# ActiveVisionLab/gaussctrl

Hardware: AMD Instinct MI355X
Metric: edited views/sec @512x512 (ControlNet denoise + splat render+bwd) (higher is better)
Workload: dtype bf16

## Files before the change

### gaussctrl_amd/csrc/dn_gemm_kernels.h

```cpp
#pragma once
#include "dn_common.h"
#include <type_traits>

namespace dng {
struct GemmArgs {
    int64_t M, N, K;
    const void *A; int64_t lda;
    int B, Hi, Wi, Cin, Ho, Wo, stride, ups, pad;
    const void *W;
    const float *bias;
    const float *rowvec; int64_t ld_rowvec; int64_t rows_per_batch;
    const void *residual; int64_t ldr;
    float out_scale;
    int act, geglu;
    void *out; int64_t ldc; int out_f32;
    void *out_t; int64_t ldt; int64_t t_batch_stride; int64_t t_col0;
    int splits; int tiles_per_split;
    int persist;
    float *ws;
    const void *zeros;
    const float *row_stats; int row_stat_slots; const float *colsum; float ln_eps, ln_inv_k;
    float *out_row_stats;
    float *out_group_stats;
    int gn_groups, gn_cpg;
// ... 887 lines not shown
            }
            block(f1, f0, st1, 0, more, tnone, std::false_type{}, w3_tag);
            st = st1;
        }
    };
    if (w3) run(std::true_type{}); else run(std::false_type{});

    if constexpr (FUSE) {
        wave_epilogue<T, NTW, MT, 512>(g, acc, m_base, m_base + wm * (16 * MT), n_base + wn * (16 * NTW), lane, smem,
                                       (g.row_stats && g.splits == 1) ? srow : nullptr, slice);
        return;
    }
    const int64_t n_lane = n_base + wn * (16 * NTW) + fc * 4;
    if (g.splits > 1) {
#pragma unroll
        for (int mt = 0; mt < MT; ++mt) {
            const int64_t m = m_base + wm * (16 * MT) + mt * 16 + fr;
            if (m >= g.M) continue;
#pragma unroll
            for (int nt = 0; nt < NTW; ++nt) {
                const int64_t n = n_lane + nt * 16;
                if (n < g.N)
                    *reinterpret_cast<float4 *>(g.ws + ((int64_t)slice * g.M + m) * g.N + n) =
                        make_float4(acc[nt][mt][0], acc[nt][mt][1], acc[nt][mt][2], acc[nt][mt][3]);
            }
        }
        return;
    }
    if constexpr (LNV == 3) {
        const float *biasp = g.bias + wset * g.N, *csp = g.colsum + wset * g.N;
        float4 bia[NTW], csm[NTW];
#pragma unroll
        for (int nt = 0; nt < NTW; ++nt) {
            const int64_t n = n_lane + nt * 16, nc = n < g.N ? n : g.N - 4;
            bia[nt] = *reinterpret_cast<const float4 *>(biasp + nc);
            csm[nt] = *reinterpret_cast<const float4 *>(csp + nc);
        }
#pragma unroll
        for (int mt = 0; mt < MT; ++mt) {
            const int64_t m = m_base + wm * (16 * MT) + mt * 16 + fr;
            const float2 st = *reinterpret_cast<const float2 *>(srow + 2 * (wm * (16 * MT) + mt * 16 + fr));
            const float mean = st.x * g.ln_inv_k, rstd = rsqrtf(fmaxf(st.y * g.ln_inv_k - mean * mean, 0.f) + g.ln_eps);
            float v[NTW][4];
            float mx = -3.0e38f;
#pragma unroll
            for (int nt = 0; nt < NTW; ++nt) {
                v[nt][0] = rstd * (acc[nt][mt][0] - mean * csm[nt].x) + bia[nt].x; v[nt][1] = rstd * (acc[nt][mt][1] - mean * csm[nt].y) + bia[nt].y;
                v[nt][2] = rstd * (acc[nt][mt][2] - mean * csm[nt].z) + bia[nt].z; v[nt][3] = rstd * (acc[nt][mt][3] - mean * csm[nt].w) + bia[nt].w;
#pragma unroll
                for (int r = 0; r < 4; ++r) {
                    const bool key = nt * 16 + fc * 4 + r < g.sm_keys;
                    v[nt][r] = key ? v[nt][r] : -3.0e38f;
                    mx = fmaxf(mx, v[nt][r]);
                }
            }
            mx = fmaxf(mx, __shfl_xor(mx, 16, 64)); mx = fmaxf(mx, __shfl_xor(mx, 32, 64));
            float sum = 0.f;
#pragma unroll
            for (int nt = 0; nt < NTW; ++nt)
#pragma unroll
                for (int r = 0; r < 4; ++r) { v[nt][r] = exp2f(v[nt][r] - mx); sum += v[nt][r]; }
            sum += __shfl_xor(sum, 16, 64); sum += __shfl_xor(sum, 32, 64);
            const float inv = 1.f / sum;
#pragma unroll
            for (int nt = 0; nt < NTW; ++nt) {
                const int64_t n = n_lane + nt * 16;
                if (m < g.M && n < g.N)
                    *reinterpret_cast<uint2 *>((unsigned char *)g.out + (m * g.ldc + n) * 2) =
                        make_uint2(pack2<T>(v[nt][0] * inv, v[nt][1] * inv), pack2<T>(v[nt][2] * inv, v[nt][3] * inv));
            }
        }
        return;
    }
    if constexpr (LEAN) {
        const unsigned char *zp = (const unsigned char *)g.zeros;
        const bool has_b = g.bias != nullptr, has_rv = g.rowvec != nullptr, has_res = g.residual != nullptr;
        const float *biasp = has_b ? g.bias + (LNV != 0 ? wset * g.N : 0) : reinterpret_cast<const float *>(zp);
        const float *rvp = has_rv ? g.rowvec : reinterpret_cast<const float *>(zp);
        const unsigned char *resp = has_res ? (const unsigned char *)g.residual : zp;
        const int64_t bA = m_base / g.rows_per_batch, b_last = (g.M - 1) / g.rows_per_batch;
        const int64_t bB = bA + 1 < b_last ? bA + 1 : b_last;
        const int64_t m_rv = (bA + 1) * g.rows_per_batch;
        float4 bia[NTW], rvA[NTW], rvB[NTW];
        uint2 rs[MT][NTW];
#pragma unroll
        for (int nt = 0; nt < NTW; ++nt) {
            const int64_t n = n_lane + nt * 16, nc = n < g.N ? n : g.N - 4;
            bia[nt] = *reinterpret_cast<const float4 *>(biasp + (has_b ? nc : 0));
            rvA[nt] = *reinterpret_cast<const float4 *>(rvp + (has_rv ? bA * g.ld_rowvec + nc : 0));
            rvB[nt] = *reinterpret_cast<const float4 *>(rvp + (has_rv ? bB * g.ld_rowvec + nc : 0));
        }
#pragma unroll
        for (int mt = 0; mt < MT; ++mt) {
            const int64_t m = m_base + wm * (16 * MT) + mt * 16 + fr, mc = m < g.M ? m : g.M - 1;
#pragma unroll
            for (int nt = 0; nt < NTW; ++nt) {
                const int64_t n = n_lane + nt * 16, nc = n < g.N ? n : g.N - 4;
                rs[mt][nt] = *reinterpret_cast<const uint2 *>(resp + (has_res ? (mc * g.ldr + nc) * 2 : 0));
            }
        }
        float4 csm[LNV == 2 ? NTW : 1];
        if constexpr (LNV == 2) {
#pragma unroll
            for (int nt = 0; nt < NTW; ++nt) {
                const int64_t n = n_lane + nt * 16, nc = n < g.N ? n : g.N - 4;
                csm[nt] = *reinterpret_cast<const float4 *>(g.colsum + wset * g.N + nc);
            }
        }
        uint2 pks[CS ? MT : 1][CS ? NTW : 1];
#pragma unroll
        for (int mt = 0; mt < MT; ++mt) {
            const int64_t m = m_base + wm * (16 * MT) + mt * 16 + fr;
            const bool second = m >= m_rv;
            float mean = 0.f, rstd = 1.f;
            if constexpr (LNV == 2) {
                const float2 st = *reinterpret_cast<const float2 *>(srow + 2 * (wm * (16 * MT) + mt * 16 + fr));
                mean = st.x * g.ln_inv_k;
                rstd = rsqrtf(fmaxf(st.y * g.ln_inv_k - mean * mean, 0.f) + g.ln_eps);
            }
            float rsum = 0.f, rsq = 0.f;
#pragma unroll
            for (int nt = 0; nt < NTW; ++nt) {
                const int64_t n = n_lane + nt * 16;
                const float4 rv = second ? rvB[nt] : rvA[nt];
                float a0 = acc[nt][mt][0], a1 = acc[nt][mt][1], a2 = acc[nt][mt][2], a3 = acc[nt][mt][3];
                if constexpr (LNV == 2) {
                    a0 = rstd * (a0 - mean * csm[nt].x); a1 = rstd * (a1 - mean * csm[nt].y);
                    a2 = rstd * (a2 - mean * csm[nt].z); a3 = rstd * (a3 - mean * csm[nt].w);
                }
                float v[4] = {a0 + bia[nt].x + rv.x, a1 + bia[nt].y + rv.y, a2 + bia[nt].z + rv.z, a3 + bia[nt].w + rv.w};
#pragma unroll
                for (int r = 0; r < 4; ++r) v[r] *= g.out_scale;
                v[0] += T::to_f((unsigned short)(rs[mt][nt].x & 0xffff)); v[1] += T::to_f((unsigned short)(rs[mt][nt].x >> 16));
                v[2] += T::to_f((unsigned short)(rs[mt][nt].y & 0xffff)); v[3] += T::to_f((unsigned short)(rs[mt][nt].y >> 16));
                const uint2 pk = make_uint2(pack2<T>(v[0], v[1]), pack2<T>(v[2], v[3]));
                const bool ok = m < g.M && n < g.N;
                if (ok) *reinterpret_cast<uint2 *>((unsigned char *)g.out + (m * g.ldc + n) * 2) = pk;
                if constexpr (CS) pks[mt][nt] = ok ? pk : make_uint2(0u, 0u);
                if constexpr (LNV == 1) {
                    const float w_ = n < g.N ? 1.f : 0.f;
                    const float t0 = w_ * T::to_f((unsigned short)(pk.x & 0xffff)), t1 = w_ * T::to_f((unsigned short)(pk.x >> 16));
                    const float t2 = w_ * T::to_f((unsigned short)(pk.y & 0xffff)), t3 = w_ * T::to_f((unsigned short)(pk.y >> 16));
                    rsum += (t0 + t1) + (t2 + t3); rsq += (t0 * t0 + t1 * t1) + (t2 * t2 + t3 * t3);
                }
            }
            if constexpr (LNV == 1) {
                rsum += __shfl_xor(rsum, 16, 64); rsq += __shfl_xor(rsq, 16, 64);
                rsum += __shfl_xor(rsum, 32, 64); rsq += __shfl_xor(rsq, 32, 64);
                const int64_t slot = (n_base + wn * (16 * NTW)) / (16 * NTW);
                if (fc == 0 && m < g.M && n_base + wn * (16 * NTW) < g.N)
                    *reinterpret_cast<float2 *>(g.out_row_stats + (slot * g.M + m) * 2) = make_float2(rsum, rsq);
            }
        }
        if constexpr (CS) {
            const int64_t m_split = (m_base / g.rows_per_batch + 1) * g.rows_per_batch;
            const int64_t m_end = m_base + BM < g.M ? m_base + BM : g.M;
            const int npass = m_split < m_end ? 2 : 1;
    #pragma unroll 1
            for (int pass = 0; pass < npass; ++pass) {
                float cs[NTW][4], cq[NTW][4];
    #pragma unroll
                for (int nt = 0; nt < NTW; ++nt)
    #pragma unroll
                    for (int r = 0; r < 4; ++r) { cs[nt][r] = 0.f; cq[nt][r] = 0.f; }
    #pragma unroll
                for (int mt = 0; mt < MT; ++mt) {
                    const int64_t m_tile = m_base + wm * (16 * MT) + mt * 16;
                    const float wgt = ((m_tile >= m_split ? 1 : 0) == pass) ? 1.f : 0.f;
    #pragma unroll
                    for (int nt = 0; nt < NTW; ++nt) {
                        const uint2 pk = pks[mt][nt];
                        const float t0 = wgt != 0.f ? T::to_f((unsigned short)(pk.x & 0xffff)) : 0.f, t1 = wgt != 0.f ? T::to_f((unsigned short)(pk.x >> 16)) : 0.f;
                        const float t2 = wgt != 0.f ? T::to_f((unsigned short)(pk.y & 0xffff)) : 0.f, t3 = wgt != 0.f ? T::to_f((unsigned short)(pk.y >> 16)) : 0.f;
                        cs[nt][0] += t0; cq[nt][0] += t0 * t0; cs[nt][1] += t1; cq[nt][1] += t1 * t1;
                        cs[nt][2] += t2; cq[nt][2] += t2 * t2; cs[nt][3] += t3; cq[nt][3] += t3 * t3;
                    }
                }
                float *tb = ctab + (pass * BN + wn * (16 * NTW) + fc * 4) * 2;
    #pragma unroll
                for (int nt = 0; nt < NTW; ++nt)
    #pragma unroll
                    for (int r = 0; r < 4; ++r) {
                        const float sa = row16_sum(cs[nt][r]), sb = row16_sum(cq[nt][r]);
                        if (fr == 0) {
                            __hip_atomic_fetch_add(tb + (nt * 16 + r) * 2, sa, __ATOMIC_RELAXED, __HIP_MEMORY_SCOPE_WORKGROUP);
                            __hip_atomic_fetch_add(tb + (nt * 16 + r) * 2 + 1, sb, __ATOMIC_RELAXED, __HIP_MEMORY_SCOPE_WORKGROUP);
                        }
                    }
            }
            asm volatile("s_waitcnt lgkmcnt(0)" ::: "memory");
            __builtin_amdgcn_s_barrier();
            const int64_t b0 = m_base / g.rows_per_batch;
            const int cpg = g.gn_cpg, G = (int)(g.N / cpg);
            const int n_hi = (int)(n_base + BN < g.N ? n_base + BN : g.N);
            const int g_first = (int)n_base / cpg, ng = (n_hi - 1) / cpg - g_first + 1;
            for (int i = tid; i < 2 * ng; i += 512) {
                const int slot = i >= ng ? 1 : 0, gg = g_first + i - slot * ng;
                if (slot == 1 && !(m_split < m_end)) continue;
                const int c_lo = gg * cpg > (int)n_base ? gg * cpg : (int)n_base, c_hi = (gg + 1) * cpg < n_hi ? (gg + 1) * cpg : n_hi;
                float s1 = 0.f, s2 = 0.f;
                for (int c = c_lo; c < c_hi; ++c) { const float2 t = *reinterpret_cast<const float2 *>(ctab + (slot * BN + c - (int)n_base) * 2); s1 += t.x; s2 += t.y; }
                const int64_t b = b0 + slot;
                const int64_t slab = mblk - (b * g.rows_per_batch) / BM;
                const int half = gg * cpg < (int)n_base ? 1 : 0;
                *reinterpret_cast<float2 *>(g.chan_parts + ((((b * g.cp_nslab + slab) * G + gg) * 2 + half) * 2)) = make_float2(s1, s2);
            }
        }
    } else {
    float4 bia[NTW], csm[LNV == 2 ? NTW : 1];
#pragma unroll
    for (int nt = 0; nt < NTW; ++nt) {
        const int64_t n = n_lane + nt * 16;
        bia[nt] = (g.bias && n < g.N) ? *reinterpret_cast<const float4 *>(g.bias + n) : make_float4(0.f, 0.f, 0.f, 0.f);
        if constexpr (LNV == 2) csm[nt] = n < g.N ? *reinterpret_cast<const float4 *>(g.colsum + n) : make_float4(0.f, 0.f, 0.f, 0.f);
    }
#pragma unroll
    for (int mt = 0; mt < MT; ++mt) {
        const int64_t m = m_base + wm * (16 * MT) + mt * 16 + fr;
        if (m >= g.M) continue;
        if constexpr (LNV == 2) {
            const float2 st = *reinterpret_cast<const float2 *>(srow + 2 * (wm * (16 * MT) + mt * 16 + fr));
            const float mean = st.x * g.ln_inv_k, rstd = rsqrtf(fmaxf(st.y * g.ln_inv_k - mean * mean, 0.f) + g.ln_eps);
#pragma unroll
            for (int nt = 0; nt < NTW; ++nt) {
                acc[nt][mt][0] = rstd * (acc[nt][mt][0] - mean * csm[nt].x); acc[nt][mt][1] = rstd * (acc[nt][mt][1] - mean * csm[nt].y);
                acc[nt][mt][2] = rstd * (acc[nt][mt][2] - mean * csm[nt].z); acc[nt][mt][3] = rstd * (acc[nt][mt][3] - mean * csm[nt].w);
            }
        }
        float4 rv[NTW];
        uint2 rs[NTW];
        const int64_t bidx = g.rowvec ? m / g.rows_per_batch : 0;
#pragma unroll
        for (int nt = 0; nt < NTW; ++nt) {
            const int64_t n = n_lane + nt * 16;
            const bool okn = n < g.N && !(g.geglu && (nt & 1));
            const int64_t on = g.geglu ? (n_base + wn * (16 * NTW) + nt * 16) / 2 + fc * 4 : n;
            rv[nt] = (g.rowvec && n < g.N) ? *reinterpret_cast<const float4 *>(g.rowvec + bidx * g.ld_rowvec + n) : make_float4(0.f, 0.f, 0.f, 0.f);
            rs[nt] = (g.residual && okn) ? *reinterpret_cast<const uint2 *>((const unsigned char *)g.residual + (m * g.ldr + on) * 2) : make_uint2(0u, 0u);
        }
#pragma unroll
        for (int nt = 0; nt < NTW; ++nt) {
            const int64_t n = n_lane + nt * 16;
            if (n >= g.N) continue;
            if (g.geglu && (nt & 1)) continue;
            float v[4] = {acc[nt][mt][0] + bia[nt].x + rv[nt].x, acc[nt][mt][1] + bia[nt].y + rv[nt].y,
                          acc[nt][mt][2] + bia[nt].z + rv[nt].z, acc[nt][mt][3] + bia[nt].w + rv[nt].w};
            int64_t on = n;
            if (g.geglu) {
                constexpr int NP = NTW - 1;
                const int np = nt + 1 < NTW ? nt + 1 : NP;
                v[0] *= gelu_erf(acc[np][mt][0] + bia[np].x); v[1] *= gelu_erf(acc[np][mt][1] + bia[np].y);
                v[2] *= gelu_erf(acc[np][mt][2] + bia[np].z); v[3] *= gelu_erf(acc[np][mt][3] + bia[np].w);
                on = (n_base + wn * (16 * NTW) + nt * 16) / 2 + fc * 4;
            }
            if (g.act == 1) {
#pragma unroll
                for (int r = 0; r < 4; ++r) v[r] = silu(v[r]);
            } else if (g.act == 2) {
#pragma unroll
                for (int r = 0; r < 4; ++r) v[r] = fminf(fmaxf(v[r] * 0.5f + 0.5f, 0.f), 1.f);
            }
#pragma unroll
            for (int r = 0; r < 4; ++r) v[r] *= g.out_scale;
            if (g.residual) {
                v[0] += T::to_f((unsigned short)(rs[nt].x & 0xffff)); v[1] += T::to_f((unsigned short)(rs[nt].x >> 16));
                v[2] += T::to_f((unsigned short)(rs[nt].y & 0xffff)); v[3] += T::to_f((unsigned short)(rs[nt].y >> 16));
            }
            const bool to_t = g.out_t && on >= g.t_col0;
            const uint2 pk = make_uint2(pack2<T>(v[0], v[1]), pack2<T>(v[2], v[3]));
            if (g.out && !(to_t && g.t_col0 > 0)) {
                if (g.out_f32)
                    *reinterpret_cast<float4 *>((float *)g.out + m * g.ldc + on) = make_float4(v[0], v[1], v[2], v[3]);
                else
                    *reinterpret_cast<uint2 *>((unsigned char *)g.out + (m * g.ldc + on) * 2) = pk;
            }
            if (to_t) {
                const int64_t b = m / g.rows_per_batch, tok = m - b * g.rows_per_batch;
                unsigned short *o = (unsigned short *)g.out_t + b * g.t_batch_stride + tok;
#pragma unroll
                for (int r = 0; r < 4; ++r) o[(on - g.t_col0 + r) * g.ldt] = T::from_f(v[r]);
            }
        }
    }
    }
}


template <class T, int NTW, int MT, int LNV = 0>
__global__ __launch_bounds__(512, 1) void k_gemm8p(const GemmArgs g)
{
    static_assert(LNV == 0 || LNV == 2, "persistent kernel: plain or LayerNorm-folded consumer");
    constexpr int BM = 64 * MT, BN = 32 * NTW, STAGE = BM * 128 + BN * 128, NS = 3;
    constexpr int AG = BM / 8, WG = BN / 8, AI = AG / 8, WI = (WG + 7) / 8;
    static_assert(WG % 8 == 0, "every wave issues the same number of W loads");
    constexpr int GRPW = AI + WI;
    extern __shared__ __attribute__((aligned(16))) unsigned char smem[];
    const int tid = threadIdx.x, lane = tid & 63;
    const int wid = __builtin_amdgcn_readfirstlane(tid >> 6);
    const int wm = wid >> 1, wn = wid & 1;
    const int nbn = (int)((g.N + BN - 1) / BN);
    const int64_t ntiles = ((g.M + BM - 1) / BM) * nbn;
    const int nk = (int)(g.K / BK);
    const unsigned lds0 = (unsigned)(size_t)(__attribute__((address_space(3))) unsigned char *)smem;
    float *srow = reinterpret_cast<float *>(smem + NS * STAGE);
    const int lr = lane >> 3, ls = lane & 7;
    const unsigned char *Ab = (const unsigned char *)g.A, *Wb = (const unsigned char *)g.W;
    auto tile_of = [&](int64_t d, int64_t &m_base, int64_t &n_base) __attribute__((always_inline)) {
        const int64_t xcd = d & 7, qq = ntiles >> 3, rr = ntiles & 7;
        const int64_t bid = (xcd < rr ? xcd * (qq + 1) : rr * (qq + 1) + (xcd - rr) * qq) + (d >> 3);
        int64_t mblk, nblk;
        dng::tile_coords(bid, (int)((g.M + BM - 1) / BM), nbn, g.pw, mblk, nblk);
        m_base = mblk * BM; n_base = nblk * BN;
    };
    int a_off[AI], w_off[WI];
    auto set_offsets = [&](int64_t m_base, int64_t n_base) __attribute__((always_inline)) {
#pragma unroll
        for (int i = 0; i < AI; ++i) {
            const int row = (wid + 8 * i) * 8 + lr;
            const int64_t m = m_base + row;
            a_off[i] = (int)(m < g.M ? m : g.M - 1) * (int)g.lda + (ls ^ ((row >> 1) & 7)) * 8;
        }
#pragma unroll
        for (int i = 0; i < WI; ++i) {
            const int row = (wid + 8 * i) * 8 + lr;
            const int64_t n = n_base + row;
            w_off[i] = (int)(n < g.N ? n : g.N - 1) * (int)g.K + (ls ^ ((row >> 1) & 7)) * 8;
        }
    };
    auto issue_a = [&](int kt, int stage, int i) __attribute__((always_inline)) {
        glds16_s(Ab + (size_t)kt * (BK * 2), (unsigned)(a_off[i] * 2), lds0 + stage * STAGE + (unsigned)((wid + 8 * i) * 1024));
    };
    auto issue_w = [&](int kt, int stage, int i) __attribute__((always_inline)) {
        glds16_s(Wb + (size_t)kt * (BK * 2), (unsigned)(w_off[i] * 2), lds0 + stage * STAGE + (unsigned)(BM * 128 + (wid + 8 * i) * 1024));
    };
    auto issue = [&](int kt, int stage) __attribute__((always_inline)) {
#pragma unroll
        for (int i = 0; i < AI; ++i) issue_a(kt, stage, i);
#pragma unroll
        for (int i = 0; i < WI; ++i) issue_w(kt, stage, i);
    };
    const int fr = lane & 15, fc = lane >> 4;
    const int swz = (fr >> 1) & 7;
    const int fx0 = ((fc ^ swz) << 4), fx1 = (((fc + 4) ^ swz) << 4);
    const int aw0 = BM * 128 + (wn * (16 * NTW) + fr) * 128, aa0 = (wm * (16 * MT) + fr) * 128;
    struct Frag { uint4 w[NTW], a[MT]; };
    auto load_frag = [&](Frag &f, int stage, int ks) __attribute__((always_inline)) {
        const unsigned char *sb = smem + stage * STAGE;
        const int fx = ks ? fx1 : fx0;
#pragma unroll
        for (int t = 0; t < NTW; ++t) f.w[t] = *reinterpret_cast<const uint4 *>(sb + aw0 + fx + t * 2048);
#pragma unroll
        for (int t = 0; t < MT; ++t) f.a[t] = *reinterpret_cast<const uint4 *>(sb + aa0 + fx + t * 2048);
    };
    f32x4 acc[NTW][MT];
    constexpr int NMM = NTW * MT, NPC = AI + WI;
    auto block = [&](const Frag &f, Frag &fn, int st_next, int ks_next, bool load_next, int dma_kt, int dma_stage, auto dma_tag) __attribute__((always_inline)) {
        constexpr bool DMA = decltype(dma_tag)::value;
        static_for<0, NMM>([&](auto m_) __attribute__((always_inline)) {
            constexpr int m = decltype(m_)::value, nt = m / MT, mt = m % MT;
            acc[nt][mt] = T::mfma(f.w[nt], f.a[mt], acc[nt][mt]);
            if constexpr (m == 0) {
                __builtin_amdgcn_sched_barrier(0);
                if (load_next) load_frag(fn, st_next, ks_next);
                __builtin_amdgcn_sched_barrier(0);
            } else if constexpr (DMA && m >= 2) {
                static_for<0, NPC>([&](auto p_) __attribute__((always_inline)) {
                    constexpr int pp = decltype(p_)::value;
                    if constexpr (m == 2 + (pp * (NMM - 3)) / NPC) {
                        __builtin_amdgcn_sched_barrier(0);
                        if constexpr (pp < AI) issue_a(dma_kt, dma_stage, pp); else issue_w(dma_kt, dma_stage, pp - AI);
                        __builtin_amdgcn_sched_barrier(0);
                    }
                });
            }
        });
    };
    auto wait_tiles = [&](auto n_) __attribute__((always_inline)) {
        asm volatile("s_waitcnt vmcnt(%0)" ::"n"(decltype(n_)::value * GRPW) : "memory");
    };

    int64_t d = blockIdx.x, m_base, n_base;
    if (d >= ntiles) return;
    tile_of(d, m_base, n_base);
    set_offsets(m_base, n_base);
    issue(0, 0);
    if (nk > 1) issue(1, 1);
    if (nk > 2) issue(2, 2);
    bool first = true;
    for (;;) {
#pragma unroll
        for (int a = 0; a < NTW; ++a)
#pragma unroll
            for (int b = 0; b < MT; ++b) acc[a][b] = f32x4{0.f, 0.f, 0.f, 0.f};
        if (first) { if (nk > 2) wait_tiles(std::integral_constant<int, 2>{}); else if (nk > 1) wait_tiles(std::integral_constant<int, 1>{}); else wait_tiles(std::integral_constant<int, 0>{}); }
        else asm volatile("s_waitcnt vmcnt(0)" ::: "memory");
        first = false;
        __builtin_amdgcn_s_barrier();
        Frag f0, f1;
        load_frag(f0, 0, 0);
        int st = 0, kt = 0;
        for (; kt + 3 < nk; ++kt) {
            const int st1 = st + 1 == NS ? 0 : st + 1;
            block(f0, f1, st, 1, true, 0, 0, std::false_type{});
            wait_tiles(std::integral_constant<int, 1>{});
            asm volatile("s_waitcnt lgkmcnt(0)" ::: "memory");
            __builtin_amdgcn_s_barrier();
            block(f1, f0, st1, 0, true, kt + 3, st, std::true_type{});
            st = st1;
        }
        for (; kt < nk; ++kt) {
            const int st1 = st + 1 == NS ? 0 : st + 1;
            block(f0, f1, st, 1, true, 0, 0, std::false_type{});
            if (kt + 1 < nk) {
                if (kt + 2 < nk) wait_tiles(std::integral_constant<int, 1>{}); else wait_tiles(std::integral_constant<int, 0>{});
                asm volatile("s_waitcnt lgkmcnt(0)" ::: "memory");
                __builtin_amdgcn_s_barrier();
                block(f1, f0, st1, 0, true, 0, 0, std::false_type{});
            } else {
                block(f1, f0, st1, 0, false, 0, 0, std::false_type{});
            }
            st = st1;
        }
        const int64_t cm = m_base, cn = n_base;
        d += gridDim.x;
        const bool more = d < ntiles;
        asm volatile("s_waitcnt lgkmcnt(0)" ::: "memory");
        __builtin_amdgcn_s_barrier();
        if constexpr (LNV == 2) {
            row_stats_prologue<BM>(g, cm, srow);
            __builtin_amdgcn_s_barrier();
        }
        if (more) {
            tile_of(d, m_base, n_base);
            set_offsets(m_base, n_base);
            issue(0, 0);
            if (nk > 1) issue(1, 1);
            if (nk > 2) issue(2, 2);
        }
        {
            const int64_t n_lane = cn + wn * (16 * NTW) + fc * 4;
            float4 bia[NTW], csm[LNV == 2 ? NTW : 1];
#pragma unroll
            for (int nt = 0; nt < NTW; ++nt) {
                const int64_t n = n_lane + nt * 16;
                bia[nt] = (g.bias && n < g.N) ? *reinterpret_cast<const float4 *>(g.bias + n) : make_float4(0.f, 0.f, 0.f, 0.f);
                if constexpr (LNV == 2) csm[nt] = n < g.N ? *reinterpret_cast<const float4 *>(g.colsum + n) : make_float4(0.f, 0.f, 0.f, 0.f);
            }
            float2 st[LNV == 2 ? MT : 1];
            if constexpr (LNV == 2) {
#pragma unroll
                for (int mt = 0; mt < MT; ++mt) st[mt] = *reinterpret_cast<const float2 *>(srow + 2 * (wm * (16 * MT) + mt * 16 + fr));
            }
#pragma unroll
            for (int mt = 0; mt < MT; ++mt) {
                const int64_t m = cm + wm * (16 * MT) + mt * 16 + fr;
                if (m >= g.M) continue;
                if constexpr (LNV == 2) {
                    const float mean = st[mt].x * g.ln_inv_k, rstd = rsqrtf(fmaxf(st[mt].y * g.ln_inv_k - mean * mean, 0.f) + g.ln_eps);
#pragma unroll
                    for (int nt = 0; nt < NTW; ++nt) {
                        acc[nt][mt][0] = rstd * (acc[nt][mt][0] - mean * csm[nt].x); acc[nt][mt][1] = rstd * (acc[nt][mt][1] - mean * csm[nt].y);
                        acc[nt][mt][2] = rstd * (acc[nt][mt][2] - mean * csm[nt].z); acc[nt][mt][3] = rstd * (acc[nt][mt][3] - mean * csm[nt].w);
                    }
                }
#pragma unroll
                for (int nt = 0; nt < NTW; ++nt) {
                    const int64_t n = n_lane + nt * 16;
                    if (n >= g.N) continue;
                    if (g.geglu && (nt & 1)) continue;
                    float v[4] = {acc[nt][mt][0] + bia[nt].x, acc[nt][mt][1] + bia[nt].y, acc[nt][mt][2] + bia[nt].z, acc[nt][mt][3] + bia[nt].w};
                    int64_t on = n;
                    if (g.geglu) {
                        constexpr int NP = NTW - 1;
                        const int np = nt + 1 < NTW ? nt + 1 : NP;
                        v[0] *= gelu_erf(acc[np][mt][0] + bia[np].x); v[1] *= gelu_erf(acc[np][mt][1] + bia[np].y);
                        v[2] *= gelu_erf(acc[np][mt][2] + bia[np].z); v[3] *= gelu_erf(acc[np][mt][3] + bia[np].w);
                        on = (cn + wn * (16 * NTW) + nt * 16) / 2 + fc * 4;
                    }
                    if (g.act == 1) {
#pragma unroll
                        for (int r = 0; r < 4; ++r) v[r] = silu(v[r]);
                    }
#pragma unroll
                    for (int r = 0; r < 4; ++r) v[r] *= g.out_scale;
                    if (g.residual) {
                        const uint2 rs = *reinterpret_cast<const uint2 *>((const unsigned char *)g.residual + (m * g.ldr + on) * 2);
                        v[0] += T::to_f((unsigned short)(rs.x & 0xffff)); v[1] += T::to_f((unsigned short)(rs.x >> 16));
                        v[2] += T::to_f((unsigned short)(rs.y & 0xffff)); v[3] += T::to_f((unsigned short)(rs.y >> 16));
                    }
                    *reinterpret_cast<uint2 *>((unsigned char *)g.out + (m * g.ldc + on) * 2) = make_uint2(pack2<T>(v[0], v[1]), pack2<T>(v[2], v[3]));
                }
            }
        }
        if (!more) break;
    }
}

template <class T, int NTW, int MT, int LNV = 0>
void launch8p(const GemmArgs &g, int nwg, hipStream_t s)
{
    constexpr size_t lds = 3 * (64 * MT * 128 + 32 * NTW * 128) + (LNV == 2 ? 64 * MT * 8 : 0);
    static_assert(lds <= 160 * 1024, "LDS ring");
    static gc::AttrOnce once;
    gc::ensure_dynamic_lds(once, (const void *)k_gemm8p<T, NTW, MT, LNV>, (int)lds);
    hipLaunchKernelGGL((k_gemm8p<T, NTW, MT, LNV>), dim3(nwg), dim3(512), lds, s, g);
}

typedef __attribute__((ext_vector_type(8))) int i32x8;

template <class T, int MODE, int NTW, int MT, bool FUSE, bool CS = false>
__global__ __launch_bounds__(512, 1) void k_gemm8q(const GemmArgs g)
{
    static_assert(MODE == 2 || MODE == 3, "fp8 path: fast conv (2) and aligned linear (3)");
    constexpr int BM = 64 * MT, BN = 32 * NTW, STAGE = BM * 128 + BN * 128, NS = 3;
    constexpr int AG = BM / 8, WG = BN / 8, AI = AG / 8, WI = (WG + 7) / 8;
    constexpr int BKB = 128;
    extern __shared__ __attribute__((aligned(16))) unsigned char smem[];
    const int tid = threadIdx.x, lane = tid & 63;
    const int wid = __builtin_amdgcn_readfirstlane(tid >> 6);
    const int wm = wid >> 1, wn = wid & 1;
    const int nbn = (int)((g.N + BN - 1) / BN);
    int64_t mblk, nblk;
    int slice;
    wg_tile(g, (int)((g.M + BM - 1) / BM), nbn, mblk, nblk, slice);
    const int64_t m_base = mblk * BM, n_base = nblk * BN;
    const int nk_all = (int)(g.K / BKB);
    const int k0 = g.splits > 1 ? slice * g.tiles_per_split : 0;
    const int nk = g.splits > 1 ? (nk_all - k0 < g.tiles_per_split ? nk_all - k0 : g.tiles_per_split) : nk_all;
    const unsigned lds0 = (unsigned)(size_t)(__attribute__((address_space(3))) unsigned char *)smem;
    float *srow = reinterpret_cast<float *>(smem + NS * STAGE);
    if constexpr (FUSE) {
        if (g.row_stats) row_stats_prologue<BM>(g, m_base, srow);
    }
    static_assert(!(FUSE && CS), "one statistics epilogue at a time");
    float *ctab = reinterpret_cast<float *>(smem + NS * STAGE);
    if constexpr (CS) {
        for (int i = tid; i < 4 * BN; i += 512) ctab[i] = 0.f;
    }
    const int lr = lane >> 3, ls = lane & 7;
    int a_off[AI];
    unsigned a_vm[AI];
    const unsigned char *a_ptr[AI];
#pragma unroll
    for (int i = 0; i < AI; ++i) {
        const int row = (wid + 8 * i) * 8 + lr;
        const int ck = ls ^ ((row >> 1) & 7);
        const int64_t m = m_base + row;
        const bool ok = m < g.M;
        a_vm[i] = 0; a_ptr[i] = (const unsigned char *)g.A; a_off[i] = 0;
        if (MODE == 2) {
            const int mm = ok ? (int)m : 0, hw = g.Ho * g.Wo, b = mm / hw, rem = mm - b * hw, oy = rem / g.Wo;
            const int y0 = oy * g.stride - g.pad, x0 = (rem - oy * g.Wo) * g.stride - g.pad;
            a_ptr[i] = (const unsigned char *)g.A + ((int64_t)(b * g.Hi + y0) * g.Wi + x0) * g.Cin + ck * 16;
            unsigned vm = 0;
#pragma unroll
            for (int tp = 0; tp < 9; ++tp) {
                const int yi = y0 + tp / 3, xi = x0 + tp % 3;
                if (ok && (unsigned)yi < (unsigned)g.Hi && (unsigned)xi < (unsigned)g.Wi) vm |= 1u << tp;
            }
            a_vm[i] = vm;
        } else {
            a_off[i] = (int)(m < g.M ? m : g.M - 1) * (int)g.lda + ck * 16;
        }
    }
    int w_off[WI];
#pragma unroll
    for (int i = 0; i < WI; ++i) {
        const int row = (wid + 8 * i) * 8 + lr;
        const int64_t n = n_base + row;
        w_off[i] = (int)(n < g.N ? n : g.N - 1) * (int)g.K + (ls ^ ((row >> 1) & 7)) * 16;
    }
    const unsigned char *Ab = (const unsigned char *)g.A, *Wb = (const unsigned char *)g.W, *Zp = (const unsigned char *)g.zeros;
    const bool tap_inner = MODE == 2 && g.conv_korder != 0;
    const KOrder kord(tap_inner, BKB, g.Cin);
    KCur cur0 = {0, 0};
    if (MODE == 2) cur0 = kord.at(k0, BKB, g.Cin);
    struct TileSrc { int kb, tap, tap_off; unsigned sbase; KCur next; };
    auto issue_begin = [&](int kt, int stage, const KCur c) __attribute__((always_inline)) -> TileSrc {
        TileSrc t;
        t.kb = (k0 + kt) * BKB; t.tap = 0; t.tap_off = 0; t.next = c;
        if (MODE == 2) {
            const int ci = kord.ci(c);
            t.tap = kord.tap(c);
            t.kb = __builtin_amdgcn_readfirstlane(t.tap * g.Cin + ci);
            const int dy = t.tap / 3, dx = t.tap - dy * 3;
            t.tap_off = (dy * g.Wi + dx) * g.Cin + ci;
            t.next = kord.next(c);
        }
        t.sbase = lds0 + stage * STAGE;
        return t;
    };
    auto issue_a = [&](const TileSrc &t, int i) __attribute__((always_inline)) {
        const unsigned dst = t.sbase + (unsigned)((wid + 8 * i) * 1024);
        if (MODE == 3) { glds16_s(Ab + (size_t)t.kb, (unsigned)a_off[i], dst); return; }
        const bool okm = (a_vm[i] >> t.tap) & 1u;
        glds16(okm ? a_ptr[i] + (int64_t)t.tap_off : Zp, dst);
    };
    auto issue_w = [&](const TileSrc &t, int i, bool has) __attribute__((always_inline)) {
        if (has) glds16_s(Wb + (size_t)t.kb, (unsigned)w_off[i], t.sbase + (unsigned)(BM * 128 + (wid + 8 * i) * 1024));
    };
    auto issue = [&](int kt, int stage, const KCur c) __attribute__((always_inline)) -> KCur {
        const TileSrc t = issue_begin(kt, stage, c);
#pragma unroll
        for (int i = 0; i < AI; ++i) issue_a(t, i);
#pragma unroll
        for (int i = 0; i < WI; ++i) issue_w(t, i, wid + 8 * i < WG);
        return t.next;
    };

    f32x4 acc[NTW][MT];
#pragma unroll
    for (int a = 0; a < NTW; ++a)
#pragma unroll
        for (int b = 0; b < MT; ++b) acc[a][b] = f32x4{0.f, 0.f, 0.f, 0.f};
    const int fr = lane & 15, fc = lane >> 4;
    const int swz = (fr >> 1) & 7;
    const int fx0 = ((fc ^ swz) << 4), fx1 = (((fc + 4) ^ swz) << 4);
    const int aw0 = BM * 128 + (wn * (16 * NTW) + fr) * 128, aa0 = (wm * (16 * MT) + fr) * 128;
    typedef __attribute__((ext_vector_type(4))) int i32x4;
    struct Frag { i32x8 w[NTW], a[MT]; };
    auto ld32 = [&](const unsigned char *p0, const unsigned char *p1) __attribute__((always_inline)) -> i32x8 {
        const i32x4 lo = *reinterpret_cast<const i32x4 *>(p0), hi = *reinterpret_cast<const i32x4 *>(p1);
        return __builtin_shufflevector(lo, hi, 0, 1, 2, 3, 4, 5, 6, 7);
    };
    auto load_frag = [&](Frag &f, int stage) __attribute__((always_inline)) {
        const unsigned char *sb = smem + stage * STAGE;
#pragma unroll
        for (int t = 0; t < NTW; ++t) f.w[t] = ld32(sb + aw0 + fx0 + t * 2048, sb + aw0 + fx1 + t * 2048);
#pragma unroll
        for (int t = 0; t < MT; ++t) f.a[t] = ld32(sb + aa0 + fx0 + t * 2048, sb + aa0 + fx1 + t * 2048);
    };
    int sw[NTW];
#pragma unroll
    for (int t = 0; t < NTW; ++t) {
        const int64_t n = n_base + wn * (16 * NTW) + t * 16 + fr;
        sw[t] = g.w_scale[n < g.N ? n : g.N - 1];
    }
    asm volatile("s_waitcnt vmcnt(0)" ::: "memory");
#pragma unroll
    for (int t = 0; t < NTW; ++t) asm volatile("" : "+v"(sw[t]));
    const int sa = g.a_scale;
    constexpr int NMM = NTW * MT, NPC = AI + WI;
    auto block = [&](const Frag &f, Frag &fn, int st_next, bool load_next, const TileSrc &t, auto dma_tag, auto w3_tag) __attribute__((always_inline)) {
        constexpr bool DMA = decltype(dma_tag)::value, W3 = decltype(w3_tag)::value;
        static_for<0, NMM>([&](auto m_) __attribute__((always_inline)) {
            constexpr int m = decltype(m_)::value, nt = m / MT, mt = m % MT;
            acc[nt][mt] = __builtin_amdgcn_mfma_scale_f32_16x16x128_f8f6f4(f.w[nt], f.a[mt], acc[nt][mt], 0, 0, 0, sw[nt], 0, sa);
            if constexpr (m == 0) {
                __builtin_amdgcn_sched_barrier(0);
                if (load_next) load_frag(fn, st_next);
                __builtin_amdgcn_sched_barrier(0);
            } else if constexpr (DMA && m >= 2) {
                static_for<0, NPC>([&](auto p_) __attribute__((always_inline)) {
                    constexpr int pp = decltype(p_)::value;
                    if constexpr (m == 2 + (pp * (NMM - 3)) / NPC) {
                        __builtin_amdgcn_sched_barrier(0);
                        if constexpr (pp < AI) issue_a(t, pp); else issue_w(t, pp - AI, (pp - AI) < WI - 1 || W3 || WG % 8 == 0);
                        __builtin_amdgcn_sched_barrier(0);
                    }
                });
            }
        });
    };
    const bool w3 = (wid + 8 * (WI - 1)) < WG;
    Frag f0, f1;
    const TileSrc tnone = {0, 0, 0, 0u, {0, 0}};
    auto run = [&](auto w3_tag) __attribute__((always_inline)) {
        constexpr bool W3 = decltype(w3_tag)::value;
        constexpr int GRPW = AI + ((W3 || WG % 8 == 0) ? WI : WI - 1);
        auto wait_tiles = [&](auto n_) __attribute__((always_inline)) {
            asm volatile("s_waitcnt vmcnt(%0)" ::"n"(decltype(n_)::value * GRPW) : "memory");
        };
        KCur cur = issue(0, 0, cur0);
        if (nk > 1) cur = issue(1, 1, cur);
        if (nk > 2) cur = issue(2, 2, cur);
        if (nk > 2) wait_tiles(std::integral_constant<int, 2>{}); else if (nk > 1) wait_tiles(std::integral_constant<int, 1>{}); else wait_tiles(std::integral_constant<int, 0>{});
        __builtin_amdgcn_s_barrier();
        load_frag(f0, 0);
        int st = 0, kt = 0;
        auto step = [&](Frag &fc_, Frag &fn_) __attribute__((always_inline)) {
            const int st1 = st + 1 == NS ? 0 : st + 1;
            if (kt + 3 < nk) {
                wait_tiles(std::integral_constant<int, 1>{});
                asm volatile("s_waitcnt lgkmcnt(0)" ::: "memory");
                __builtin_amdgcn_s_barrier();
                const TileSrc t = issue_begin(kt + 3, st, cur);
                cur = t.next;
                block(fc_, fn_, st1, true, t, std::true_type{}, w3_tag);
            } else {
                const bool more = kt + 1 < nk;
                if (more) {
                    if (kt + 2 < nk) wait_tiles(std::integral_constant<int, 1>{}); else wait_tiles(std::integral_constant<int, 0>{});
                    asm volatile("s_waitcnt lgkmcnt(0)" ::: "memory");
                    __builtin_amdgcn_s_barrier();
                }
                block(fc_, fn_, st1, more, tnone, std::false_type{}, w3_tag);
            }
            st = st1; ++kt;
        };
        while (kt < nk) {
            step(f0, f1);
            if (kt < nk) step(f1, f0);
        }
    };
    if (w3) run(std::true_type{}); else run(std::false_type{});
    if constexpr (FUSE) {
        wave_epilogue<T, NTW, MT, 512>(g, acc, m_base, m_base + wm * (16 * MT), n_base + wn * (16 * NTW), lane, smem, g.row_stats ? srow : nullptr, slice);
        return;
    }
    const int64_t n_lane = n_base + wn * (16 * NTW) + fc * 4;
    if (g.splits > 1) {
#pragma unroll
        for (int mt = 0; mt < MT; ++mt) {
            const int64_t m = m_base + wm * (16 * MT) + mt * 16 + fr;
            if (m >= g.M) continue;
#pragma unroll
            for (int nt = 0; nt < NTW; ++nt) {
                const int64_t n = n_lane + nt * 16;
                if (n < g.N)
                    *reinterpret_cast<float4 *>(g.ws + ((int64_t)slice * g.M + m) * g.N + n) =
                        make_float4(acc[nt][mt][0], acc[nt][mt][1], acc[nt][mt][2], acc[nt][mt][3]);
            }
        }
        return;
    }
    if constexpr (CS) {
        const unsigned char *zp = (const unsigned char *)g.zeros;
        const bool has_b = g.bias != nullptr, has_rv = g.rowvec != nullptr, has_res = g.residual != nullptr;
        const float *biasp = has_b ? g.bias : reinterpret_cast<const float *>(zp);
        const float *rvp = has_rv ? g.rowvec : reinterpret_cast<const float *>(zp);
        const unsigned char *resp = has_res ? (const unsigned char *)g.residual : zp;
        const int64_t bA = m_base / g.rows_per_batch, b_last = (g.M - 1) / g.rows_per_batch;
        const int64_t bB = bA + 1 < b_last ? bA + 1 : b_last;
        const int64_t m_rv = (bA + 1) * g.rows_per_batch;
        float4 bia[NTW], rvA[NTW], rvB[NTW];
        uint2 rs[MT][NTW];
#pragma unroll
        for (int nt = 0; nt < NTW; ++nt) {
            const int64_t n = n_lane + nt * 16, nc = n < g.N ? n : g.N - 4;
            bia[nt] = *reinterpret_cast<const float4 *>(biasp + (has_b ? nc : 0));
            rvA[nt] = *reinterpret_cast<const float4 *>(rvp + (has_rv ? bA * g.ld_rowvec + nc : 0));
            rvB[nt] = *reinterpret_cast<const float4 *>(rvp + (has_rv ? bB * g.ld_rowvec + nc : 0));
        }
#pragma unroll
        for (int mt = 0; mt < MT; ++mt) {
            const int64_t m = m_base + wm * (16 * MT) + mt * 16 + fr, mc = m < g.M ? m : g.M - 1;
#pragma unroll
            for (int nt = 0; nt < NTW; ++nt) {
                const int64_t n = n_lane + nt * 16, nc = n < g.N ? n : g.N - 4;
                rs[mt][nt] = *reinterpret_cast<const uint2 *>(resp + (has_res ? (mc * g.ldr + nc) * 2 : 0));
            }
        }
        uint2 pks[MT][NTW];
#pragma unroll
        for (int mt = 0; mt < MT; ++mt) {
            const int64_t m = m_base + wm * (16 * MT) + mt * 16 + fr;
            const bool second = m >= m_rv;
#pragma unroll
            for (int nt = 0; nt < NTW; ++nt) {
                const int64_t n = n_lane + nt * 16;
                const float4 rv = second ? rvB[nt] : rvA[nt];
                float v[4] = {acc[nt][mt][0] + bia[nt].x + rv.x, acc[nt][mt][1] + bia[nt].y + rv.y,
                              acc[nt][mt][2] + bia[nt].z + rv.z, acc[nt][mt][3] + bia[nt].w + rv.w};
#pragma unroll
                for (int r = 0; r < 4; ++r) v[r] *= g.out_scale;
                v[0] += T::to_f((unsigned short)(rs[mt][nt].x & 0xffff)); v[1] += T::to_f((unsigned short)(rs[mt][nt].x >> 16));
                v[2] += T::to_f((unsigned short)(rs[mt][nt].y & 0xffff)); v[3] += T::to_f((unsigned short)(rs[mt][nt].y >> 16));
                const uint2 pk = make_uint2(pack2<T>(v[0], v[1]), pack2<T>(v[2], v[3]));
                const bool ok = m < g.M && n < g.N;
                if (ok) *reinterpret_cast<uint2 *>((unsigned char *)g.out + (m * g.ldc + n) * 2) = pk;
                pks[mt][nt] = ok ? pk : make_uint2(0u, 0u);
            }
        }
        {
            const int64_t m_split = (m_base / g.rows_per_batch + 1) * g.rows_per_batch;
            const int64_t m_end = m_base + BM < g.M ? m_base + BM : g.M;
            const int npass = m_split < m_end ? 2 : 1;
    #pragma unroll 1
            for (int pass = 0; pass < npass; ++pass) {
                float cs[NTW][4], cq[NTW][4];
    #pragma unroll
                for (int nt = 0; nt < NTW; ++nt)
    #pragma unroll
                    for (int r = 0; r < 4; ++r) { cs[nt][r] = 0.f; cq[nt][r] = 0.f; }
    #pragma unroll
                for (int mt = 0; mt < MT; ++mt) {
                    const int64_t m_tile = m_base + wm * (16 * MT) + mt * 16;
                    const float wgt = ((m_tile >= m_split ? 1 : 0) == pass) ? 1.f : 0.f;
    #pragma unroll
                    for (int nt = 0; nt < NTW; ++nt) {
                        const uint2 pk = pks[mt][nt];
                        const float t0 = wgt != 0.f ? T::to_f((unsigned short)(pk.x & 0xffff)) : 0.f, t1 = wgt != 0.f ? T::to_f((unsigned short)(pk.x >> 16)) : 0.f;
                        const float t2 = wgt != 0.f ? T::to_f((unsigned short)(pk.y & 0xffff)) : 0.f, t3 = wgt != 0.f ? T::to_f((unsigned short)(pk.y >> 16)) : 0.f;
                        cs[nt][0] += t0; cq[nt][0] += t0 * t0; cs[nt][1] += t1; cq[nt][1] += t1 * t1;
                        cs[nt][2] += t2; cq[nt][2] += t2 * t2; cs[nt][3] += t3; cq[nt][3] += t3 * t3;
                    }
                }
                float *tb = ctab + (pass * BN + wn * (16 * NTW) + fc * 4) * 2;
    #pragma unroll
                for (int nt = 0; nt < NTW; ++nt)
    #pragma unroll
                    for (int r = 0; r < 4; ++r) {
                        const float sa = row16_sum(cs[nt][r]), sb = row16_sum(cq[nt][r]);
                        if (fr == 0) {
// ... 405 lines not shown
```

Before: 11.33.

## Overlap persistent GEMM epilogue with next tile's prefetch and LN stats

The persistent bf16 GEMM now stages bias and colsum for each column tile into double-buffered LDS via DMA. LayerNorm row statistics for the next tile are loaded and folded into a double-buffered LDS slot during the current tile's epilogue, replacing a separate prologue and barrier between tiles. Residual loads are hoisted ahead of the math, and output stores are deferred until after a single vmcnt wait. The first K-steps of the next tile skip the explicit vmcnt waits because the epilogue already drained them. This hides epilogue latency at the cost of more LDS, more registers and fragile wait-count bookkeeping.

```diff
diff --git a/gaussctrl_amd/csrc/dn_gemm_kernels.h b/gaussctrl_amd/csrc/dn_gemm_kernels.h
--- a/gaussctrl_amd/csrc/dn_gemm_kernels.h
+++ b/gaussctrl_amd/csrc/dn_gemm_kernels.h
@@ -1213,8 +1213,10 @@
     const int64_t ntiles = ((g.M + BM - 1) / BM) * nbn;
     const int nk = (int)(g.K / BK);
     const unsigned lds0 = (unsigned)(size_t)(__attribute__((address_space(3))) unsigned char *)smem;
+    static_assert(BN == 128, "ecol: one 16-byte DMA per lane of one wave covers bias | colsum of the column tile");
+    constexpr int SROW_BYTES = LNV == 2 ? 2 * BM * 8 : 0, ECOL_BYTES = 2 * BN * 4;
     float *srow = reinterpret_cast<float *>(smem + NS * STAGE);
-    const int lr = lane >> 3, ls = lane & 7;
+    const float *ecol = reinterpret_cast<const float *>(smem + NS * STAGE + SROW_BYTES);
     const unsigned char *Ab = (const unsigned char *)g.A, *Wb = (const unsigned char *)g.W;
     auto tile_of = [&](int64_t d, int64_t &m_base, int64_t &n_base) __attribute__((always_inline)) {
         const int64_t xcd = d & 7, qq = ntiles >> 3, rr = ntiles & 7;
@@ -1224,7 +1226,8 @@
         m_base = mblk * BM; n_base = nblk * BN;
     };
     int a_off[AI], w_off[WI];
-    auto set_offsets = [&](int64_t m_base, int64_t n_base) __attribute__((always_inline)) {
+    auto set_offsets = [&](int t, int64_t m_base, int64_t n_base) __attribute__((always_inline)) {
+        const int lr = (t & 63) >> 3, ls = t & 7;
 #pragma unroll
         for (int i = 0; i < AI; ++i) {
             const int row = (wid + 8 * i) * 8 + lr;
@@ -1290,13 +1293,76 @@
         asm volatile("s_waitcnt vmcnt(%0)" ::"n"(decltype(n_)::value * GRPW) : "memory");
     };
 
+    auto stage_cols = [&](int t, int64_t n_base, int h) __attribute__((always_inline)) {
+        if (wid == 0) {
+            const int64_t n = n_base + (t & 31) * 4;
+            const float *src = (t & 63) < 32 ? g.bias : (LNV == 2 ? g.colsum : nullptr);
+            const void *p = (src && n < g.N) ? (const void *)(src + n) : g.zeros;
+            glds16(p, lds0 + (unsigned)(NS * STAGE + SROW_BYTES + h * ECOL_BYTES));
+        }
+    };
+    constexpr int PF = 11;
+    auto stats_issue = [&](float2 (&P)[PF], int t, int64_t m_base) __attribute__((always_inline)) {
+        const int r = t & 255, hf = t >> 8;
+        if (r < BM) {
+            const int64_t m = m_base + r < g.M ? m_base + r : g.M - 1;
+            const float *rp = g.row_stats + m * 2;
+            const int64_t st = g.M * 2;
+#pragma unroll
+            for (int j = 0; j < PF; ++j) {
+                const int sl = hf + 2 * j;
+                P[j] = *reinterpret_cast<const float2 *>(rp + (sl < g.row_stat_slots ? sl : g.row_stat_slots - 1) * st);
+            }
+        }
+    };
+    auto stats_fold = [&](const float2 (&P)[PF], int t, int64_t m_base, float *dst) __attribute__((always_inline)) {
+        const int r = t & 255, hf = t >> 8;
+        if (r < BM) {
+            const int nh = (g.row_stat_slots - hf + 1) >> 1;
+            float sx = 0.f, sy = 0.f;
+            int i = 0;
+            static_for<0, 2>([&](auto g_) __attribute__((always_inline)) {
+                constexpr int q = 4 * decltype(g_)::value;
+                if (q + 4 <= nh) {
+                    sx += (P[q].x + P[q + 1].x) + (P[q + 2].x + P[q + 3].x); sy += (P[q].y + P[q + 1].y) + (P[q + 2].y + P[q + 3].y);
+                    i = q + 4;
+                }
+            });
+            if (nh > PF) {
+                const int64_t m = m_base + r < g.M ? m_base + r : g.M - 1;
+                const float *rp = g.row_stats + m * 2 + hf * g.M * 2;
+                const int64_t st = g.M * 4;
+                for (; i + 4 <= nh; i += 4) {
+                    const float2 a = *reinterpret_cast<const float2 *>(rp + i * st), b = *reinterpret_cast<const float2 *>(rp + (i + 1) * st);
+                    const float2 c = *reinterpret_cast<const float2 *>(rp + (i + 2) * st), e = *reinterpret_cast<const float2 *>(rp + (i + 3) * st);
+                    sx += (a.x + b.x) + (c.x + e.x); sy += (a.y + b.y) + (c.y + e.y);
+                }
+                for (; i < nh; ++i) {
+                    const float2 a = *reinterpret_cast<const float2 *>(rp + i * st);
+                    sx += a.x; sy += a.y;
+                }
+            } else {
+                static_for<0, PF>([&](auto j_) __attribute__((always_inline)) {
+                    constexpr int j = decltype(j_)::value;
+                    if (j >= i && j < nh) { sx += P[j].x; sy += P[j].y; }
+                });
+            }
+            __hip_atomic_fetch_add(dst + 2 * r, sx, __ATOMIC_RELAXED, __HIP_MEMORY_SCOPE_WORKGROUP);
+            __hip_atomic_fetch_add(dst + 2 * r + 1, sy, __ATOMIC_RELAXED, __HIP_MEMORY_SCOPE_WORKGROUP);
+        }
+        asm volatile("s_waitcnt lgkmcnt(0)" ::: "memory");
+    };
+
     int64_t d = blockIdx.x, m_base, n_base;
     if (d >= ntiles) return;
     tile_of(d, m_base, n_base);
-    set_offsets(m_base, n_base);
+    set_offsets(tid, m_base, n_base);
+    int eb = 0, sb = 0;
+    stage_cols(tid, n_base, 0);
     issue(0, 0);
     if (nk > 1) issue(1, 1);
     if (nk > 2) issue(2, 2);
+    if constexpr (LNV == 2) row_stats_prologue<BM>(g, m_base, srow);
     bool first = true;
     for (;;) {
 #pragma unroll
@@ -1304,12 +1370,20 @@
 #pragma unroll
             for (int b = 0; b < MT; ++b) acc[a][b] = f32x4{0.f, 0.f, 0.f, 0.f};
         if (first) { if (nk > 2) wait_tiles(std::integral_constant<int, 2>{}); else if (nk > 1) wait_tiles(std::integral_constant<int, 1>{}); else wait_tiles(std::integral_constant<int, 0>{}); }
-        else asm volatile("s_waitcnt vmcnt(0)" ::: "memory");
+        const int npre = first ? 0 : 2;
         first = false;
         __builtin_amdgcn_s_barrier();
         Frag f0, f1;
         load_frag(f0, 0, 0);
         int st = 0, kt = 0;
+        for (; kt < npre && kt + 3 < nk; ++kt) {
+            const int st1 = st + 1 == NS ? 0 : st + 1;
+            block(f0, f1, st, 1, true, 0, 0, std::false_type{});
+            asm volatile("s_waitcnt lgkmcnt(0)" ::: "memory");
+            __builtin_amdgcn_s_barrier();
+            block(f1, f0, st1, 0, true, kt + 3, st, std::true_type{});
+            st = st1;
+        }
         for (; kt + 3 < nk; ++kt) {
             const int st1 = st + 1 == NS ? 0 : st + 1;
             block(f0, f1, st, 1, true, 0, 0, std::false_type{});
@@ -1323,7 +1397,7 @@
             const int st1 = st + 1 == NS ? 0 : st + 1;
             block(f0, f1, st, 1, true, 0, 0, std::false_type{});
             if (kt + 1 < nk) {
-                if (kt + 2 < nk) wait_tiles(std::integral_constant<int, 1>{}); else wait_tiles(std::integral_constant<int, 0>{});
+                if (kt >= npre) { if (kt + 2 < nk) wait_tiles(std::integral_constant<int, 1>{}); else wait_tiles(std::integral_constant<int, 0>{}); }
                 asm volatile("s_waitcnt lgkmcnt(0)" ::: "memory");
                 __builtin_amdgcn_s_barrier();
                 block(f1, f0, st1, 0, true, 0, 0, std::false_type{});
@@ -1335,38 +1409,45 @@
         const int64_t cm = m_base, cn = n_base;
         d += gridDim.x;
         const bool more = d < ntiles;
+        if (more) tile_of(d, m_base, n_base);
+        const bool flip = LNV == 2 && more && m_base != cm;
+        int te = tid;
+        asm volatile("" : "+v"(te));
+        const int fre = te & 15, fce = (te >> 4) & 3;
+        if (flip && te < 2 * BM) srow[(sb ^ 1) * (2 * BM) + te] = 0.f;
         asm volatile("s_waitcnt lgkmcnt(0)" ::: "memory");
         __builtin_amdgcn_s_barrier();
-        if constexpr (LNV == 2) {
-            row_stats_prologue<BM>(g, cm, srow);
-            __builtin_amdgcn_s_barrier();
-        }
         if (more) {
-            tile_of(d, m_base, n_base);
-            set_offsets(m_base, n_base);
+            set_offsets(te, m_base, n_base);
+            stage_cols(te, n_base, eb ^ 1);
             issue(0, 0);
             if (nk > 1) issue(1, 1);
             if (nk > 2) issue(2, 2);
         }
+        float2 P[PF];
+        if constexpr (LNV == 2) {
+            __builtin_amdgcn_sched_barrier(0);
+            stats_issue(P, te, m_base);
+            __builtin_amdgcn_sched_barrier(0);
+        }
         {
-            const int64_t n_lane = cn + wn * (16 * NTW) + fc * 4;
+            const int64_t n_lane = cn + wn * (16 * NTW) + fce * 4;
+            const float *ec = ecol + eb * (2 * BN) + wn * (16 * NTW) + fce * 4;
             float4 bia[NTW], csm[LNV == 2 ? NTW : 1];
 #pragma unroll
             for (int nt = 0; nt < NTW; ++nt) {
-                const int64_t n = n_lane + nt * 16;
-                bia[nt] = (g.bias && n < g.N) ? *reinterpret_cast<const float4 *>(g.bias + n) : make_float4(0.f, 0.f, 0.f, 0.f);
-                if constexpr (LNV == 2) csm[nt] = n < g.N ? *reinterpret_cast<const float4 *>(g.colsum + n) : make_float4(0.f, 0.f, 0.f, 0.f);
+                bia[nt] = *reinterpret_cast<const float4 *>(ec + nt * 16);
+                if constexpr (LNV == 2) csm[nt] = *reinterpret_cast<const float4 *>(ec + BN + nt * 16);
             }
             float2 st[LNV == 2 ? MT : 1];
             if constexpr (LNV == 2) {
 #pragma unroll
-                for (int mt = 0; mt < MT; ++mt) st[mt] = *reinterpret_cast<const float2 *>(srow + 2 * (wm * (16 * MT) + mt * 16 + fr));
-            }
-#pragma unroll
-            for (int mt = 0; mt < MT; ++mt) {
-                const int64_t m = cm + wm * (16 * MT) + mt * 16 + fr;
-                if (m >= g.M) continue;
-                if constexpr (LNV == 2) {
+                for (int mt = 0; mt < MT; ++mt) st[mt] = *reinterpret_cast<const float2 *>(srow + sb * (2 * BM) + 2 * (wm * (16 * MT) + mt * 16 + fre));
+            }
+            uint2 pk[MT][NTW];
+            if constexpr (LNV == 2) {
+#pragma unroll
+                for (int mt = 0; mt < MT; ++mt) {
                     const float mean = st[mt].x * g.ln_inv_k, rstd = rsqrtf(fmaxf(st[mt].y * g.ln_inv_k - mean * mean, 0.f) + g.ln_eps);
 #pragma unroll
                     for (int nt = 0; nt < NTW; ++nt) {
@@ -1374,19 +1455,29 @@
                         acc[nt][mt][2] = rstd * (acc[nt][mt][2] - mean * csm[nt].z); acc[nt][mt][3] = rstd * (acc[nt][mt][3] - mean * csm[nt].w);
                     }
                 }
+            }
+#pragma unroll
+            for (int mt = 0; mt < MT; ++mt) {
+                uint2 rs[NTW];
+                if (g.residual) {
+                    const int64_t m = cm + wm * (16 * MT) + mt * 16 + fre;
+#pragma unroll
+                    for (int nt = 0; nt < NTW; ++nt) {
+                        const int64_t n = n_lane + nt * 16;
+                        const int64_t on = g.geglu ? (cn + wn * (16 * NTW) + nt * 16) / 2 + fce * 4 : n;
+                        const bool ok = m < g.M && n < g.N && !(g.geglu && (nt & 1));
+                        rs[nt] = ok ? *reinterpret_cast<const uint2 *>((const unsigned char *)g.residual + (m * g.ldr + on) * 2) : make_uint2(0u, 0u);
+                    }
+                }
 #pragma unroll
                 for (int nt = 0; nt < NTW; ++nt) {
-                    const int64_t n = n_lane + nt * 16;
-                    if (n >= g.N) continue;
                     if (g.geglu && (nt & 1)) continue;
                     float v[4] = {acc[nt][mt][0] + bia[nt].x, acc[nt][mt][1] + bia[nt].y, acc[nt][mt][2] + bia[nt].z, acc[nt][mt][3] + bia[nt].w};
-                    int64_t on = n;
                     if (g.geglu) {
                         constexpr int NP = NTW - 1;
                         const int np = nt + 1 < NTW ? nt + 1 : NP;
                         v[0] *= gelu_erf(acc[np][mt][0] + bia[np].x); v[1] *= gelu_erf(acc[np][mt][1] + bia[np].y);
                         v[2] *= gelu_erf(acc[np][mt][2] + bia[np].z); v[3] *= gelu_erf(acc[np][mt][3] + bia[np].w);
-                        on = (cn + wn * (16 * NTW) + nt * 16) / 2 + fc * 4;
                     }
                     if (g.act == 1) {
 #pragma unroll
@@ -1395,22 +1486,41 @@
 #pragma unroll
                     for (int r = 0; r < 4; ++r) v[r] *= g.out_scale;
                     if (g.residual) {
-                        const uint2 rs = *reinterpret_cast<const uint2 *>((const unsigned char *)g.residual + (m * g.ldr + on) * 2);
-                        v[0] += T::to_f((unsigned short)(rs.x & 0xffff)); v[1] += T::to_f((unsigned short)(rs.x >> 16));
-                        v[2] += T::to_f((unsigned short)(rs.y & 0xffff)); v[3] += T::to_f((unsigned short)(rs.y >> 16));
+                        v[0] += T::to_f((unsigned short)(rs[nt].x & 0xffff)); v[1] += T::to_f((unsigned short)(rs[nt].x >> 16));
+                        v[2] += T::to_f((unsigned short)(rs[nt].y & 0xffff)); v[3] += T::to_f((unsigned short)(rs[nt].y >> 16));
                     }
-                    *reinterpret_cast<uint2 *>((unsigned char *)g.out + (m * g.ldc + on) * 2) = make_uint2(pack2<T>(v[0], v[1]), pack2<T>(v[2], v[3]));
+                    pk[mt][nt] = make_uint2(pack2<T>(v[0], v[1]), pack2<T>(v[2], v[3]));
+                    asm volatile("" : "+v"(pk[mt][nt].x), "+v"(pk[mt][nt].y));
                 }
+                __builtin_amdgcn_sched_barrier(0);
+            }
+            asm volatile("s_waitcnt vmcnt(0)" ::: "memory");
+            if constexpr (LNV == 2) {
+#pragma unroll
+                for (int j = 0; j < PF; ++j) asm volatile("" :: "v"(P[j].x), "v"(P[j].y));
+                if (flip) { stats_fold(P, te, m_base, srow + (sb ^ 1) * (2 * BM)); sb ^= 1; }
+            }
+#pragma unroll
+            for (int mt = 0; mt < MT; ++mt) {
+                const int64_t m = cm + wm * (16 * MT) + mt * 16 + fre;
+#pragma unroll
+                for (int nt = 0; nt < NTW; ++nt) {
+                    const int64_t n = n_lane + nt * 16;
+                    if (g.geglu && (nt & 1)) continue;
+                    const int64_t on = g.geglu ? (cn + wn * (16 * NTW) + nt * 16) / 2 + fce * 4 : n;
+                    if (m < g.M && n < g.N) *reinterpret_cast<uint2 *>((unsigned char *)g.out + (m * g.ldc + on) * 2) = pk[mt][nt];
+                }
             }
         }
         if (!more) break;
+        eb ^= 1;
     }
 }
 
 template <class T, int NTW, int MT, int LNV = 0>
 void launch8p(const GemmArgs &g, int nwg, hipStream_t s)
 {
-    constexpr size_t lds = 3 * (64 * MT * 128 + 32 * NTW * 128) + (LNV == 2 ? 64 * MT * 8 : 0);
+    constexpr size_t lds = 3 * (64 * MT * 128 + 32 * NTW * 128) + (LNV == 2 ? 2 * 64 * MT * 8 : 0) + 2 * (2 * 32 * NTW * 4);
     static_assert(lds <= 160 * 1024, "LDS ring");
     static gc::AttrOnce once;
     gc::ensure_dynamic_lds(once, (const void *)k_gemm8p<T, NTW, MT, LNV>, (int)lds);
```

Result: no change. 11.33 (median of 2 runs) (+0.0%).
